# li-kunyi/CUT3R-SLAM

Measured on AMD Instinct MI355X. Metric: frames/sec (ViT pointmap + covisibility-graph tracking step) on 640x480, higher is better.
Workload: dtype f16

## Files before the change

### cut3r_slam_amd/_lib.py

```python
from __future__ import annotations

import ctypes as C
import os

_HERE = os.path.dirname(os.path.abspath(__file__))
LIB_PATH = os.path.join(_HERE, "libcut3r_hip.so")

c_void_p, c_int, c_float, c_ll = C.c_void_p, C.c_int, C.c_float, C.c_longlong


class GemmDesc(C.Structure):
    _fields_ = [
        ("A", c_void_p), ("B", c_void_p), ("C", c_void_p), ("bias", c_void_p), ("res1", c_void_p), ("res2", c_void_p),
        ("M", c_int), ("N", c_int), ("K", c_int), ("lda", c_int), ("ldb", c_int), ("ldc", c_int), ("ldr1", c_int),
        ("ldr2", c_int),
        ("act", c_int), ("out_f16", c_int), ("res1_f16", c_int), ("res2_f16", c_int),
        ("batch", c_int),
        ("strideA", c_ll), ("strideB", c_ll), ("strideC", c_ll), ("strideBias", c_ll), ("strideR1", c_ll),
        ("strideR2", c_ll),
        ("conv_k", c_int), ("H", c_int), ("W", c_int), ("Cin", c_int), ("conv_stride", c_int), ("Ho", c_int),
        ("Wo", c_int), ("relu_in", c_int),
        ("shuf", c_int), ("shuf_cout", c_int), ("shuf_Hin", c_int), ("shuf_Win", c_int),
        ("tile", c_int), ("stages", c_int),
        ("rope_pos", c_void_p), ("rope_table", c_void_p), ("rope_cols", c_int), ("rope_pmin", c_int), ("rope_npos", c_int),
# ... 3 lines not shown
    ]


class LcTerm(C.Structure):
    _fields_ = [("a", c_void_p), ("c", c_void_p), ("mask", c_void_p), ("ia", c_int), ("ic", c_int), ("w", c_float), ("pad", c_int)]


SIGNATURES = {
    "cut3r_abi_version": [],
    "cut3r_rope2d": [c_void_p, c_int, c_void_p, c_int, c_int, c_int, c_int, c_ll, c_ll, c_ll, c_float, c_float, c_void_p],
    "cut3r_rope2d_qk": [c_void_p, c_void_p, c_int, c_void_p, c_int, c_int, c_int, c_int, c_ll, c_ll, c_ll, c_ll, c_float, c_float,
                        c_void_p],
    "cut3r_rope2d_tab": [c_void_p, c_void_p, c_ll, c_ll, c_void_p, c_void_p, c_ll, c_ll, c_int, c_int, c_void_p, c_int, c_int, c_float,
                         c_float, c_void_p],
    "cut3r_layernorm": [c_void_p, c_int, c_void_p, c_void_p, c_float, c_int, c_int, c_void_p, c_int, c_void_p, c_int,
                        c_void_p, c_void_p, c_void_p],
    "cut3r_layernorm_dual": [c_void_p, c_int, c_void_p, c_void_p, c_void_p, c_int, c_void_p, c_void_p, c_void_p, c_int, c_float, c_int,
                             c_int, c_void_p],
    "cut3r_gemm_f16": [C.POINTER(GemmDesc), c_void_p],
    "cut3r_gemm_tile_for": [C.POINTER(GemmDesc)],
    "cut3r_gemm_f16_pair": [C.POINTER(GemmDesc), C.POINTER(GemmDesc), c_void_p],
    "cut3r_rope2d_table": [c_void_p, c_int, c_int, c_int, c_float, c_float, c_void_p],
    "cut3r_gemv_f16w": [c_void_p, c_int, c_void_p, c_int, c_void_p, c_void_p, c_int, c_int, c_int, c_int, c_int,
                        c_void_p, c_int, c_int, c_void_p],
    "cut3r_attention_variant": [c_int],
    "cut3r_attention_f16": [c_void_p, c_void_p, c_void_p, c_void_p, c_int, c_int, c_int, c_int, c_int,
                            c_ll, c_ll, c_ll, c_ll, c_ll, c_ll, c_ll, c_ll, c_float, c_void_p],
    "cut3r_im2col_patch": [c_void_p, c_int, c_int, c_int, c_int, c_int, c_int, c_void_p, c_void_p],
    "cut3r_cast_f32_f16": [c_void_p, c_int, c_void_p, c_int, c_int, c_int, c_void_p],
    "cut3r_colmean": [c_void_p, c_int, c_int, c_int, c_void_p, c_void_p],
    "cut3r_colmean_batched": [c_void_p, c_int, c_ll, c_int, c_int, c_int, c_void_p, c_ll, c_void_p],
    "cut3r_upsample2x_nhwc": [c_void_p, c_void_p, c_int, c_int, c_int, c_int, c_void_p],
    "cut3r_dpt_final": [c_void_p, c_int, c_int, c_void_p, c_void_p, c_int, c_void_p, c_void_p, c_void_p],
    "cut3r_postprocess_pts": [c_void_p, c_int, c_int, c_int, c_void_p, c_void_p, c_void_p],
    "cut3r_postprocess_pose": [c_void_p, c_int, c_void_p, c_void_p],
    "cut3r_patch_overlap": [c_void_p, c_void_p, c_int, c_int, c_float, c_void_p, c_void_p, c_void_p],
    "cut3r_patch_overlap_chain": [c_void_p, c_void_p, c_int, c_int, c_int, c_float, C.c_double, c_void_p, c_void_p, c_void_p, c_void_p,
                                  c_void_p, c_void_p],
    "cut3r_overlap_fwd": [c_void_p, c_int, C.POINTER(c_float), c_float, c_void_p, c_int, c_float, c_float, c_float, c_float,
                          c_int, c_int, c_int, c_void_p, c_void_p],
    "cut3r_overlap_bwd": [c_void_p, c_int, c_int, c_int, c_int, c_void_p, c_float, c_float, c_float, c_float, c_int, c_int,
                          c_void_p, c_void_p],
    "cut3r_window_update": [c_void_p, c_void_p, c_int, c_int, c_int, C.POINTER(c_float), c_float, c_int, c_void_p, c_void_p, c_void_p,
                            c_void_p, c_int, c_int, c_void_p, C.POINTER(c_float), c_int, c_int, c_float, c_float, c_float, c_float,
                            c_void_p, c_int, c_void_p, c_void_p],
    "cut3r_logdepth_accum": [c_void_p, c_void_p, c_int, c_void_p, c_void_p],
    "cut3r_resize_linear_u8": [c_void_p, c_int, c_int, c_int, c_void_p, c_int, c_int, c_int, c_void_p],
    "cut3r_mfma_probe": [c_void_p, c_int, c_int, c_int, c_void_p, c_void_p, c_void_p],
    "cut3r_remap_linear_u8": [c_void_p, c_int, c_int, c_int, c_void_p, c_void_p, c_void_p, c_int, c_int, c_void_p],
    "cut3r_align_view": [c_void_p, c_void_p, c_int, c_int, C.POINTER(c_float), c_float, c_int, c_void_p, c_void_p,
                         c_void_p, c_void_p],
    "cut3r_logdepth_sum": [c_void_p, c_void_p, c_int, c_void_p, c_void_p],
    "cut3r_lie_unary": [c_int, c_int, c_void_p, c_void_p, c_int, c_void_p],
    "cut3r_lie_unary_bwd": [c_int, c_int, c_void_p, c_void_p, c_void_p, c_int, c_void_p],
    "cut3r_lie_mul": [c_int, c_void_p, c_void_p, c_void_p, c_int, c_void_p],
    "cut3r_lie_mul_bwd": [c_int, c_void_p, c_void_p, c_void_p, c_void_p, c_void_p, c_int, c_void_p],
    "cut3r_lie_act": [c_int, c_void_p, c_void_p, c_void_p, c_int, c_int, c_int, c_void_p],
    "cut3r_lie_act_bwd": [c_int, c_void_p, c_void_p, c_void_p, c_void_p, c_void_p, c_int, c_int, c_int, c_void_p],
    "cut3r_lie_adj": [c_int, c_void_p, c_void_p, c_void_p, c_int, c_int, c_void_p],
    "cut3r_lc_workspace_floats": [c_int, c_int],
    "cut3r_lc_optimize": [c_void_p, c_void_p, c_ll, c_void_p, c_void_p, c_void_p, c_int, c_int, c_ll, c_int, c_float,
                          c_void_p, c_void_p, c_void_p, c_void_p, c_void_p, c_void_p, c_void_p],
    "cut3r_lc_optimize_terms": [c_void_p, c_int, c_int, c_int, c_int, c_float, c_void_p, c_void_p, c_void_p, c_void_p, c_void_p, c_void_p,
                                c_void_p],
    "cut3r_transform_submaps": [c_void_p, c_void_p, c_int, c_ll, c_void_p],
    "cut3r_corr_index_forward": [c_void_p, c_void_p, c_void_p, c_int, c_int, c_int, c_int, c_int, c_int, c_void_p],
# ... 85 lines not shown
```

### cut3r_slam_amd/csrc/elementwise.hip

```cpp
#include "common.h"
#include "../../include/cut3r_hip.h"

namespace {

template <typename T> struct alignas(4 * sizeof(T)) Vec4 { T v[4]; };

template <typename T>
__global__ __launch_bounds__(256) void rope2d_kernel(T* __restrict__ tok, T* __restrict__ tok2, const int64_t* __restrict__ pos,
                                                     int N, int H, int D, long long sB, long long sN, long long sH, long long sB2,
                                                     long long sN2, float base, float fwd) {
    __shared__ float cs[2][2][64];
    const int t = blockIdx.x;
    const int b = t / N, n = t - b * N;
    const int Q = D >> 2;
    if (threadIdx.x < 2 * Q) {
        const int X = threadIdx.x / Q, q = threadIdx.x - X * Q;
        const float inv = fwd / powf(base, (float)q / (float)Q);
        const float fr = (float)pos[(size_t)t * 2 + X] * inv;
        cs[X][0][q] = cosf(fr);
        cs[X][1][q] = sinf(fr);
    }
    __syncthreads();
    const int Q4 = Q >> 2;
    const int per_tensor = H * 2 * Q4;
    const int total = tok2 ? 2 * per_tensor : per_tensor;
    for (int w = threadIdx.x; w < total; w += blockDim.x) {
        const int which = w / per_tensor;
        int r = w - which * per_tensor;
        const int h = r / (2 * Q4);
        r -= h * 2 * Q4;
        const int X = r / Q4, c = r - X * Q4;
        T* base_p = which ? (tok2 + (size_t)b * sB2 + (size_t)n * sN2) : (tok + (size_t)b * sB + (size_t)n * sN);
        T* pu = base_p + (size_t)h * sH + X * 2 * Q + 4 * c;
// ... 360 lines not shown
        } else {
            const float eps = 1e-6f;
            float o[3] = {a0, a1, a2};
#pragma unroll
            for (int e = 0; e < 3; e++) {
                float sg = 1.0f / (1.0f + expf(-o[e]));
                pts[3 * p + e] = ((sg * (1 - 2 * eps) + eps) - 0.5f) * 2.0f;
            }
        }
    }
}

__global__ __launch_bounds__(256) void dpt_final_coalesced_kernel(const h16* __restrict__ in, int P, int Cin, const float* __restrict__ w,
                                                                  const float* __restrict__ bsv, int mode, float* __restrict__ pts,
                                                                  float* __restrict__ conf) {
    const int nout = mode == 0 ? 4 : 3;
    const int lane = threadIdx.x & 63;
    const int lpp = Cin >> 3;
    const int ppw = 64 / lpp;
    const int sub = lane / lpp, chunk = lane - sub * lpp;
    float wr[4][8];
#pragma unroll
    for (int o = 0; o < 4; o++)
#pragma unroll
        for (int e = 0; e < 8; e++) wr[o][e] = o < nout ? w[o * Cin + chunk * 8 + e] : 0.f;
    const float b0 = bsv[0], b1 = bsv[1], b2 = bsv[2], b3 = nout == 4 ? bsv[3] : 0.f;
    const size_t wave_global = (blockIdx.x * (size_t)blockDim.x + threadIdx.x) >> 6;
    const size_t nwaves = ((size_t)gridDim.x * blockDim.x) >> 6;
    for (size_t p0 = wave_global * ppw; p0 < (size_t)P; p0 += nwaves * ppw) {
        const size_t p = p0 + sub;
        float a0 = 0.f, a1 = 0.f, a2 = 0.f, a3 = 0.f;
        if (p < (size_t)P) {
            const half8_t v = *reinterpret_cast<const half8_t*>(in + p * Cin + chunk * 8);
#pragma unroll
            for (int e = 0; e < 8; e++) {
                const float xv = (float)v[e];
                a0 = fmaf(xv, wr[0][e], a0);
                a1 = fmaf(xv, wr[1][e], a1);
                a2 = fmaf(xv, wr[2][e], a2);
                a3 = fmaf(xv, wr[3][e], a3);
            }
        }
        for (int o = lpp >> 1; o > 0; o >>= 1) {
            a0 += __shfl_xor(a0, o, 64);
            a1 += __shfl_xor(a1, o, 64);
            a2 += __shfl_xor(a2, o, 64);
            a3 += __shfl_xor(a3, o, 64);
        }
        if (chunk == 0 && p < (size_t)P) {
            a0 += b0; a1 += b1; a2 += b2; a3 += b3;
            if (mode == 0) {
                act_pts_conf(a0, a1, a2, a3, true, false, pts, conf, p);
            } else {
                const float eps = 1e-6f;
                const float o3[3] = {a0, a1, a2};
#pragma unroll
                for (int e = 0; e < 3; e++) {
                    const float sg = 1.0f / (1.0f + expf(-o3[e]));
                    pts[3 * p + e] = ((sg * (1 - 2 * eps) + eps) - 0.5f) * 2.0f;
                }
            }
        }
    }
}

__global__ __launch_bounds__(256) void postprocess_pts_kernel(const float* __restrict__ raw, int P, int nch, int pos_z,
                                                              float* __restrict__ pts, float* __restrict__ conf) {
    for (size_t p = blockIdx.x * (size_t)blockDim.x + threadIdx.x; p < (size_t)P; p += (size_t)gridDim.x * blockDim.x) {
        const float* r = raw + p * nch;
        act_pts_conf(r[0], r[1], r[2], nch > 3 ? r[3] : 0.f, nch > 3, pos_z != 0, pts, conf, p);
    }
}

__global__ void postprocess_pose_kernel(const float* __restrict__ raw, int B, float* __restrict__ out) {
    const int b = blockIdx.x * blockDim.x + threadIdx.x;
    if (b >= B) return;
    const float* r = raw + b * 7;
    const float d = sqrtf(r[0] * r[0] + r[1] * r[1] + r[2] * r[2]);
    const float sc = expm1f(d) / fmaxf(d, 1e-8f);
    float qn = sqrtf(r[3] * r[3] + r[4] * r[4] + r[5] * r[5] + r[6] * r[6]);
    qn = fmaxf(qn, 1e-12f);
    float q[4] = {r[3] / qn, r[4] / qn, r[5] / qn, r[6] / qn};
    const float sg = q[0] < 0.f ? -1.f : 1.f;
    out[b * 7 + 0] = r[0] * sc; out[b * 7 + 1] = r[1] * sc; out[b * 7 + 2] = r[2] * sc;
    for (int e = 0; e < 4; e++) out[b * 7 + 3 + e] = sg * q[e];
// ... 241 lines not shown
```

### cut3r_slam_amd/csrc/gemm.hip

```cpp
#include <cstdlib>
#include "common.h"
#include "../../include/cut3r_hip.h"

namespace {

constexpr int BK = 64;
constexpr int KCH = BK / 8;

struct GemmArgs {
    const h16* A; const h16* B; void* C;
    const float* bias; const void* res1; const void* res2;
    int M, N, K, lda, ldb, ldc, ldr1, ldr2;
    int act, out_f16, res1_f16, res2_f16;
    long long sA, sB, sC, sBias, sR1, sR2;
    int conv_k, H, W, Cin, cstride, Ho, Wo, relu_in;
    int shuf, shuf_cout, shuf_Hin, shuf_Win;
    int swz;
    int prio;
    const long long* rope_pos; const float* rope_table; int rope_cols, rope_pmin, rope_npos, rope_d;
    const float* ln_stats; const float* ln_c; int ln_nslab; float ln_eps;
    float* stats_out; h16* out16; int ld16;
};

DEVINL half8_t relu8(half8_t v) {
#pragma unroll
    for (int i = 0; i < 8; i++) v[i] = v[i] > (h16)0 ? v[i] : (h16)0;
    return v;
}

__device__ __attribute__((aligned(16))) unsigned char g_zero16[16];

template <int N>
DEVINL void wait_vmcnt() { asm volatile("s_waitcnt vmcnt(%0)" ::"n"(N) : "memory"); }
template <int NL, int MAXF>
DEVINL void wait_tiles_in_flight(int fl) {
    static_assert(MAXF * NL <= 63, "vmcnt is a 6-bit counter");
    if constexpr (MAXF >= 6) { if (fl >= 6) { wait_vmcnt<6 * NL>(); return; } }
    if constexpr (MAXF >= 5) { if (fl == 5) { wait_vmcnt<5 * NL>(); return; } }
    if constexpr (MAXF >= 4) { if (fl == 4) { wait_vmcnt<4 * NL>(); return; } }
    if constexpr (MAXF >= 3) { if (fl == 3) { wait_vmcnt<3 * NL>(); return; } }
    if constexpr (MAXF >= 2) { if (fl == 2) { wait_vmcnt<2 * NL>(); return; } }
    if constexpr (MAXF >= 1) { if (fl == 1) { wait_vmcnt<NL>(); return; } }
    wait_vmcnt<0>();
}

DEVINL f32x4 load_res4(const void* res, int is_f16, size_t off) {
    if (is_f16) {
        const half4_t rv = *reinterpret_cast<const half4_t*>((const h16*)res + off);
        return f32x4{(float)rv[0], (float)rv[1], (float)rv[2], (float)rv[3]};
    }
    return *reinterpret_cast<const f32x4*>((const float*)res + off);
}
DEVINL f32x4 fused_finish4(const GemmArgs& g, f32x4 v, const f32x4& b4, bool has_bias, const f32x4& r1, const f32x4& r2) {
    if (has_bias) v += b4;
// ... 331 lines not shown
                fb[j] = *reinterpret_cast<const half8_t*>(sb + r * (BK * 2) + ((ch ^ (r & 7)) << 4));
            }
            if (g.prio) __builtin_amdgcn_s_setprio(1);
#pragma unroll
            for (int i = 0; i < MT; i++)
#pragma unroll
                for (int j = 0; j < NT; j++)
                    acc[i][j] = __builtin_amdgcn_mfma_f32_16x16x32_f16(fa[i], fb[j], acc[i][j], 0, 0, 0);
            if (g.prio) __builtin_amdgcn_s_setprio(0);
        }
        if (++stage == NSTAGE) stage = 0;
    }
    __syncthreads();

    float* cs = reinterpret_cast<float*>(smem);
    const float* lnp = reinterpret_cast<const float*>(smem + LNP_OFF);
    if (g.ln_stats && tid < BM) {
        float* w = reinterpret_cast<float*>(smem + LNP_OFF) + 2 * tid;
        w[0] = ln_rs; w[1] = ln_rm;
    }
    const float* bias = g.bias ? g.bias + (size_t)z * g.sBias : nullptr;
    constexpr int TPR = BN / 4;
    constexpr int RPP = NTHR / TPR;
    constexpr int ITER = (EPI_ROWS + RPP - 1) / RPP;
    constexpr int PF = (MT * NT >= 12) ? 2 : (ITER < 4 ? ITER : 4);
    const int c4 = (tid % TPR) * 4;
    const int gn = n0 + c4;
    const int r0 = tid / TPR;
    const bool col_ok = gn < N && tid < RPP * TPR;
    const bool plain = !g.shuf && g.rope_cols == 0;
    const f32x4 zero4 = {0.f, 0.f, 0.f, 0.f};
    f32x4 b4 = zero4;
    if (bias && col_ok && plain) b4 = *reinterpret_cast<const f32x4*>(bias + gn);
    if constexpr (EPI != 0) {
        constexpr bool F16OUT = EPI != 3, RES = (EPI == 3 || EPI == 5);
        const int gnc = col_ok ? gn : 0;
        const f32x4 bb = *reinterpret_cast<const f32x4*>(bias + gnc);
#pragma unroll
        for (int p = 0; p < EPI_PASSES; p++) {
            f32x4 rv[ITER], sv[ITER];
            if (RES) {
#pragma unroll
                for (int i = 0; i < ITER; i++) {
                    const size_t gm = (size_t)min(m0 + p * EPI_ROWS + r0 + i * RPP, M - 1);
                    if (EPI == 3) {
                        rv[i] = *reinterpret_cast<const f32x4*>((const float*)g.res1 + (size_t)z * g.sR1 + gm * g.ldr1 + gnc);
                    } else {
                        const half4_t h1 = *reinterpret_cast<const half4_t*>((const h16*)g.res1 + (size_t)z * g.sR1 + gm * g.ldr1 + gnc);
                        rv[i] = f32x4{(float)h1[0], (float)h1[1], (float)h1[2], (float)h1[3]};
                        if (g.res2) {
                            const half4_t h2 = *reinterpret_cast<const half4_t*>((const h16*)g.res2 + (size_t)z * g.sR2 + gm * g.ldr2 + gnc);
                            sv[i] = f32x4{(float)h2[0], (float)h2[1], (float)h2[2], (float)h2[3]};
                        }
                    }
                }
            }
            if (p > 0) __syncthreads();
#pragma unroll
            for (int i = 0; i < MT; i++)
#pragma unroll
                for (int j = 0; j < NT; j++)
#pragma unroll
                    for (int e = 0; e < 4; e++) {
                        const int r = wm * WM + i * 16 + fq * 4 + e - p * EPI_ROWS;
                        const int c = wn * WN + j * 16 + fr;
                        if (EPI_PASSES == 1 || (r >= 0 && r < EPI_ROWS)) cs[r * CPAD + c] = acc[i][j][e];
// ... 1013 lines not shown
            if (ep == 3 && ns8 == 6) hipLaunchKernelGGL((gemm_kernel<64, 64, 6, 2, 4, 1, 3>), grid, dim3(512), 0, s, g);
            else if (ep == 3 && ns8 == 4) hipLaunchKernelGGL((gemm_kernel<64, 64, 4, 2, 4, 1, 3>), grid, dim3(512), 0, s, g);
            else if (ep == 3) hipLaunchKernelGGL((gemm_kernel<64, 64, 3, 2, 4, 1, 3>), grid, dim3(512), 0, s, g);
            else if (am == 1) hipLaunchKernelGGL((gemm_kernel<64, 64, 3, 2, 4, 1>), grid, dim3(512), 0, s, g);
            else if (am == 2) hipLaunchKernelGGL((gemm_kernel<64, 64, 3, 2, 4, 2>), grid, dim3(512), 0, s, g);
            else hipLaunchKernelGGL((gemm_kernel<64, 64, 3, 2, 4>), grid, dim3(512), 0, s, g);
        }
        else if (d->stages == 4) hipLaunchKernelGGL((gemm_kernel<64, 64, 4>), grid, dim3(256), 0, s, g);
        else {
            const int am = d->stages == 0 ? tile_addr_mode(g) : 0;
            const int ep = am == 1 ? gemm256_epi_mode(g) : 0;
            if (g.stats_out && ep != 3) return CUT3R_ERR_ARG;
            static const int ns4 = [] { const char* e = getenv("CUT3R_GEMM64_STAGES"); return e ? atoi(e) : 3; }();
#define CUT3R_T64(NS)                                                                                                   \
    do {                                                                                                                 \
        if (ep == 1) hipLaunchKernelGGL((gemm_kernel<64, 64, NS, 2, 2, 1, 1>), grid, dim3(256), 0, s, g);                \
        else if (ep == 2) hipLaunchKernelGGL((gemm_kernel<64, 64, NS, 2, 2, 1, 2>), grid, dim3(256), 0, s, g);           \
        else if (ep == 3) hipLaunchKernelGGL((gemm_kernel<64, 64, NS, 2, 2, 1, 3>), grid, dim3(256), 0, s, g);           \
        else hipLaunchKernelGGL((gemm_kernel<64, 64, NS, 2, 2, 1>), grid, dim3(256), 0, s, g);                           \
    } while (0)
            if (am == 1 && ns4 == 6) CUT3R_T64(6);
            else if (am == 1 && ns4 == 4) CUT3R_T64(4);
            else if (am == 1) CUT3R_T64(3);
#undef CUT3R_T64
            else if (am == 2) hipLaunchKernelGGL((gemm_kernel<64, 64, 3, 2, 2, 2>), grid, dim3(256), 0, s, g);
            else hipLaunchKernelGGL((gemm_kernel<64, 64, 3>), grid, dim3(256), 0, s, g);
        }
    } else {
        return CUT3R_ERR_ARG;
    }
    return cut3r_check_launch();
}

extern "C" int cut3r_gemm_f16_pair(const cut3r_gemm_desc* d0, const cut3r_gemm_desc* d1, void* stream) {
    if (!d0 || !d1) return CUT3R_ERR_ARG;
    GemmPairArgs a;
    int rc = fill_args(d0, a.p[0]);
    if (rc != CUT3R_OK) return rc;
    rc = fill_args(d1, a.p[1]);
    if (rc != CUT3R_OK) return rc;
    for (const cut3r_gemm_desc* d : {d0, d1})
        if (d->conv_k == 3 || d->shuf || d->relu_in || (d->batch > 1)) return CUT3R_ERR_ARG;
    if (d0->N != d1->N || d0->K != d1->K) return CUT3R_ERR_ARG;
    hipStream_t s = (hipStream_t)stream;
    const bool special = d0->ln_stats || d1->ln_stats || d0->stats_out || d1->stats_out || a.p[0].rope_cols || a.p[1].rope_cols;
    int tile = d0->tile;
    if (tile == 0) {
        const long long t256 = (long long)((d0->M + 255) / 256 + (d1->M + 255) / 256) * ((d0->N + 255) / 256);
        const long long rounds = (t256 + 255) / 256;
        const bool fills = rounds == 1 || t256 * 100 >= rounds * 256 * 85;
        const long long t128 = (long long)((d0->M + 127) / 128 + (d1->M + 127) / 128) * ((d0->N + 127) / 128);
        tile = ((d0->N & 255) == 0 && t256 >= 128 && fills && !special) ? 256 : ((t128 >= 128 && !special) ? 128 : 64);
    }
    if (special && tile != 64) return CUT3R_ERR_ARG;
    if (tile == 64) {
        const int n0 = ((d0->N + 63) / 64) * ((d0->M + 63) / 64), n1 = ((d1->N + 63) / 64) * ((d1->M + 63) / 64);
        a.nblk0 = n0;
        a.p[0].swz = a.p[1].swz = 1;
        const bool am = tile_addr_mode(a.p[0]) == 1 && tile_addr_mode(a.p[1]) == 1;
        const int e0 = gemm256_epi_mode(a.p[0]), e1 = gemm256_epi_mode(a.p[1]);
        const int ep = (am && e0 == e1 && (e0 == 1 || e0 == 2 || e0 == 3)) ? e0 : 0;
        if ((d0->stats_out || d1->stats_out) && ep != 3) return CUT3R_ERR_ARG;
        const dim3 grid(n0 + n1);
        if (d0->K >= 2048) {
            if (ep == 3) hipLaunchKernelGGL((gemm_pair_kernel<64, 64, 3, 2, 4, 1, 3>), grid, dim3(512), 0, s, a);
            else if (am) hipLaunchKernelGGL((gemm_pair_kernel<64, 64, 3, 2, 4, 1, 0>), grid, dim3(512), 0, s, a);
// ... 36 lines not shown
```

### cut3r_slam_amd/model.py

```python
from __future__ import annotations

import gc

import math
import re
from dataclasses import dataclass
from typing import Dict, List, Optional

import torch

from . import ops
from .config import Cut3rConfig, production_config, state_dict_schema

F16, F32 = torch.float16, torch.float32


@dataclass
class ARCroco3DStereoOutput:
    ress: Optional[List[dict]] = None
    views: Optional[List[dict]] = None


class _Lin:

# ... 6 lines not shown
            w2 = torch.cat([w2, torch.zeros(pad, w2.shape[1])], 0)
            if b is not None:
                b = torch.cat([b.to(F32), torch.zeros(pad)], 0)
        self.w = w2.to(device=dev, dtype=F16).contiguous()
        self.b = b.to(device=dev, dtype=F32).contiguous() if b is not None else None
        self.npad = n + pad
        self.k = self.w.shape[1]


class Cut3rModel:
    def __init__(self, cfg: Cut3rConfig, state_dict: Dict[str, torch.Tensor], device="cuda:0", minimal: bool = False):
        self.cfg = cfg
        self.device = torch.device(device)
        self.minimal = minimal
        schema = state_dict_schema(cfg)
        missing = [k for k in schema if k not in state_dict]
        if missing:
            raise KeyError(f"state_dict is missing {len(missing)} tensors, e.g. {missing[:4]}")
        for k, shp in schema.items():
            if tuple(state_dict[k].shape) != tuple(shp):
                raise ValueError(f"{k}: shape {tuple(state_dict[k].shape)} != schema {tuple(shp)}")
        self._buf: Dict[tuple, torch.Tensor] = {}
        self._graphs: Dict[tuple, tuple] = {}
        import os as _os
        self.use_graphs = _os.environ.get("CUT3R_GRAPHS", "1") != "0"
        self.dual_stream = _os.environ.get("CUT3R_DUAL_STREAM", "1") != "0"
        self.dual_ln = _os.environ.get("CUT3R_DUAL_LN", "1") != "0"
        self.pair_gemm = _os.environ.get("CUT3R_PAIR_GEMM", "0") != "0"
        self.pair_rows = int(_os.environ.get("CUT3R_PAIR_ROWS", "0"))
        self.fused_rope = int(_os.environ.get("CUT3R_FUSED_ROPE", "1"))
        self.rope48_rows = int(_os.environ.get("CUT3R_ROPE48_ROWS", "0"))
        self.head_overlap = _os.environ.get("CUT3R_HEAD_OVERLAP", "1") != "0"
        self.head_chunk = max(1, int(_os.environ.get("CUT3R_HEAD_CHUNK", "28")))
        self.ln_fold = int(_os.environ.get("CUT3R_LN_FOLD", "1"))
        self._head_stream = None
        self._side = None
        self._head_side = None
        self.kv_fork = _os.environ.get("CUT3R_KV_FORK", "0") != "0"
        self.kv_fork_rows = int(_os.environ.get("CUT3R_KV_FORK_ROWS", "2048"))
        self._kv_streams = None
        self._prep(state_dict)

    @classmethod
    def from_state_dict(cls, cfg, sd, device="cuda:0", **kw):
        return cls(cfg, sd, device, **kw)

    @classmethod
    def from_pretrained(cls, path: str, config: Optional[Cut3rConfig] = None, device="cuda:0", **kw):
        import argparse
        import os
        if not os.path.isfile(path):
            raise FileNotFoundError(f"{path}: no checkpoint (this runtime never fetches from a hub)")
        with torch.serialization.safe_globals([argparse.Namespace]):
            ckpt = torch.load(path, map_location="cpu", weights_only=True)
        sd = ckpt["model"] if "model" in ckpt else ckpt
        sd = {(k[7:] if k.startswith("module.") else k): v for k, v in sd.items()}
        if not any(k.startswith("dec_blocks_state") for k in sd):
            for k in list(sd):
                if k.startswith("dec_blocks"):
                    sd[k.replace("dec_blocks", "dec_blocks_state")] = sd[k]
        if config is None:
            config = production_config()
            args = getattr(ckpt.get("args", None), "model", "") if isinstance(ckpt, dict) else ""
            config = _config_from_ctor_string(args, config)
        return cls(config, sd, device, **kw)

# ... 459 lines not shown
        B, H, W, _ = x.shape
        Ho, Wo = (H - 1) // stride + 1, (W - 1) // stride + 1
        out = self.buf(tag or name, (B, Ho, Wo, L.npad), F16)
        return ops.conv3x3_nhwc(x, L.w, out, L.b, stride, relu_in, act, res1, res2)

    def _conv1(self, x, name, tag=None):
        L = self.w[name]
        B, H, W, Cc = x.shape
        out = self.buf(tag or name, (B, H, W, L.npad), F16)
        ops.linear(x.view(-1, Cc), L.w, out.view(-1, L.npad), L.b)
        return out

    def _convT(self, x, name):
        L = self.w[name]
        B, H, W, Cc = x.shape
        cout = L.npad // (L.s * L.s)
        out = self.buf(name, (B, H * L.s, W * L.s, cout), F16)
        return ops.conv_transpose_nhwc(x, L.w, out, L.b, L.s)

    def _up2(self, x, tag):
        B, H, W, Cc = x.shape
        return ops.upsample2x(x, self.buf(tag, (B, 2 * H, 2 * W, Cc), F16))

    def _rcu(self, x, p, res2=None):
        t = self._conv3(x, p + ".conv1", relu_in=True, act=2)
        return self._conv3(t, p + ".conv2", res1=x, res2=res2)

    def _fusion(self, p, x0, x1=None):
        out = x0 if x1 is None else self._rcu(x1, p + ".resConfUnit1", res2=x0)
        out = self._rcu(out, p + ".resConfUnit2")
        out = self._up2(out, p + ".up")
        return self._conv1(out, p + ".out_conv")

    def _dpt(self, p, toks16: List[torch.Tensor], B, nh, nw):
        a = p + ".act_postprocess"
        t = [x.view(B, nh, nw, -1) for x in toks16]
        l0 = self._convT(self._conv1(t[0], a + ".0.0"), a + ".0.1")
        l1 = self._convT(self._conv1(t[1], a + ".1.0"), a + ".1.1")
        l2 = self._conv1(t[2], a + ".2.0")
        l3 = self._conv3(self._conv1(t[3], a + ".3.0"), a + ".3.1", stride=2)
        L = [self._conv3(l, f"{p}.scratch.layer_rn.{i}") for i, l in enumerate((l0, l1, l2, l3))]
        p4 = self._fusion(p + ".scratch.refinenet4", L[3])
        if p4.shape[1] != L[2].shape[1] or p4.shape[2] != L[2].shape[2]:
            p4 = p4[:, : L[2].shape[1], : L[2].shape[2]].contiguous()
        p3 = self._fusion(p + ".scratch.refinenet3", p4, L[2])
        p2 = self._fusion(p + ".scratch.refinenet2", p3, L[1])
        p1 = self._fusion(p + ".scratch.refinenet1", p2, L[0])
        o = self._conv3(p1, p + ".head.0")
        o = self._up2(o, p + ".head.up")
        o = self._conv3(o, p + ".head.2", act=2)
        return o

    def _dpt_pts(self, p, toks16, B, nh, nw, H, W, key_pts, key_conf, res, out=None):
        o = self._dpt(p, toks16, B, nh, nw)
        if out is None:
            pts = torch.empty((B, H, W, 3), dtype=F32, device=self.device)
            conf = torch.empty((B, H, W), dtype=F32, device=self.device)
        else:
            pts, conf = out
        ops.dpt_final(o.view(B * H * W, -1), self.w[p + ".head.4.w"], self.w[p + ".head.4.b"], 0, pts, conf)
        if res is not None:
            res[key_pts], res[key_conf] = pts, conf

    @torch.no_grad()
    def forward_window(self, imgs: torch.Tensor, return_taps: bool = False):
        if self.use_graphs and not return_taps:
            return self._graphed("win", lambda x: self._forward_window(x, False), imgs.contiguous())
        return self._forward_window(imgs, return_taps)

    @torch.no_grad()
    def encode_batch(self, imgs: torch.Tensor) -> torch.Tensor:
        if self.use_graphs:
            feat, _, _ = self._graphed("enc", self._encode, imgs.contiguous())
            return feat.clone()
        return self._encode(imgs)[0]

    @torch.no_grad()
    def decode_window(self, feats: torch.Tensor, H: int, W: int):
        if self.use_graphs:
            return self._graphed(("dec", H, W), lambda f: self._forward_window(None, False, feats=f, hw=(H, W)), feats.contiguous())
        return self._forward_window(None, False, feats=feats, hw=(H, W))

    def _forward_window(self, imgs, return_taps: bool = False, feats=None, hw=None):
        P = self.cfg.patch_size
        if feats is None:
            V, _, H, W = imgs.shape
            feat, feat16, _ = self._encode(imgs)
            res, taps = self._decode(feat[None], feat16[None], H, W, return_taps)
        else:
            H, W = hw
            res, taps = self._decode(feats[None], None, H, W, return_taps)
            V = feats.shape[0]
        preds = [{k: v[i:i + 1] for k, v in res.items()} for i in range(V)]
# ... 117 lines not shown
                        self._dec_block("decs", f"dec_blocks_state.{l}", s_a, a, pos_state, pos_img, cfg.state_dec_num_heads, s_b, Wn, pre_ln=pre,
                                        xs=xsa, ys=xa, os_=xsb)
                        self._dec_block("deci", f"dec_blocks.{l}", a, s_a, pos_img, pos_state, cfg.dec_num_heads, b, Wn, pre_ln=pre, xs=xa, ys=xsa, os_=xb)
                s_a, s_b = s_b, s_a
                a, b = b, a
                if l + 1 == h1 or l + 1 == h2:
                    tk = tok1 if l + 1 == h1 else tok2
                    tk[:, i].copy_(a.view(Wn, N + 1, D)[:, 1:])
            if not dead_tail:
                self._ln(s_a, "dec_norm_state", out32=s_b)
            new_state = s_b
            self._ln(a, "dec_norm", out16=dn16, out32=dn32)
            dn16v, dn32v = dn16.view(Wn, N + 1, D), dn32.view(Wn, N + 1, D)
            tok3[:, i].copy_(dn16v[:, 1:])
            if tok3_32 is not None:
                tok3_32[:, i].copy_(dn32v[:, 1:])
            pose_tok[:, i].copy_(dn32v[:, 0])
            pose_tok16[:, i].copy_(dn16v[:, 0])
            if not dead_tail:
                self._mem_update(mem[cm], g16, dn32v[:, 0], mem[cm ^ 1], Wn)
                cm ^= 1
            if head_fork:
                cur = torch.cuda.current_stream()
                self._head_stream.wait_stream(cur)
                with torch.cuda.stream(self._head_stream):
                    for c0 in range(0, Wn, self.head_chunk):
                        c1 = min(Wn, c0 + self.head_chunk)
                        nb = c1 - c0
                        tk = []
                        for name, src, dim in (("f", feat16, E), ("t1", tok1, D), ("t2", tok2, D), ("t3", tok3, D)):
                            t = self.buf("head.view." + name, (nb, N, dim), F16)
                            t.copy_(src[c0:c1, i])
                            tk.append(t.view(nb * N, dim))
                        pv = self.buf("head.view.pts", (nb, H, W, 3), F32)
                        cv = self.buf("head.view.conf", (nb, H, W), F32)
                        self._dpt_pts("downstream_head.dpt_self", tk, nb, nh, nw, H, W, None, None, None, out=(pv, cv))
                        head_pts.view(Wn, V, H, W, 3)[c0:c1, i].copy_(pv)
                        head_conf.view(Wn, V, H, W)[c0:c1, i].copy_(cv)
            cs = 0 if new_state is st[0] else 1
            if return_taps:
                states.append((new_state.view(Wn, S, D)[0].clone(), mem[cm].view(Wn, msz, 2 * D)[0].clone()))
        if return_taps:
            taps["states"] = states

        BV = Wn * V
        h = "downstream_head"
        ph = self.buf("head.pose_h", (BV, self.w[h + ".pose_head.mlp.fc1"].npad), F16)
        self._linear(pose_tok16.view(BV, D), h + ".pose_head.mlp.fc1", ph, act=1)
        praw = self.buf("head.pose_raw", (BV, 8), F32)
        self._linear(ph, h + ".pose_head.mlp.fc2", praw)
        pose = torch.empty((BV, 7), dtype=F32, device=dev)
        ops.postprocess_pose(praw[:, :7].contiguous(), pose)
        res: Dict[str, torch.Tensor] = {"camera_pose": pose}
        toks = [feat16.reshape(BV * N, E), tok1.view(BV * N, D), tok2.view(BV * N, D), tok3.view(BV * N, D)]
        if head_fork:
            torch.cuda.current_stream().wait_stream(self._head_stream)
            res["pts3d_in_self_view"], res["conf_self"] = head_pts, head_conf
        elif cfg.head_type == "dpt":
            pts = torch.empty((BV, H, W, 3), dtype=F32, device=dev)
            conf = torch.empty((BV, H, W), dtype=F32, device=dev)
            for c0 in range(0, BV, 8):
                c1 = min(BV, c0 + 8)
                tk = [t.view(BV, N, -1)[c0:c1].reshape((c1 - c0) * N, -1) for t in toks]
                self._dpt_pts(h + ".dpt_self", tk, c1 - c0, nh, nw, H, W, None, None, None, out=(pts[c0:c1], conf[c0:c1]))
            res["pts3d_in_self_view"], res["conf_self"] = pts, conf
        else:
            self._linear_head(h + ".proj", tok3.view(BV * N, D), BV, nh, nw, True, "pts3d_in_self_view", "conf_self", res)
        if not self.minimal:
            posBV = pos1.expand(BV, -1, -1).contiguous()
            self._cross_heads(toks, tok3_32.view(BV, N, D), pose_tok.view(BV, D), posBV, BV, nh, nw, H, W, res)
        return res, taps
# ... 112 lines not shown
```

### cut3r_slam_amd/ops.py

```python
from __future__ import annotations

import ctypes as C
import os
from typing import Optional

import torch

from . import _lib
from ._lib import GemmDesc, check

F16, F32 = torch.float16, torch.float32


def _stream():
    return C.c_void_p(torch.cuda.current_stream().cuda_stream)


def _p(t: Optional[torch.Tensor]):
    return C.c_void_p(t.data_ptr()) if t is not None else C.c_void_p(0)


def _req(cond, msg):
    if not cond:
        raise ValueError(msg)
# ... 262 lines not shown
    if bias is not None:
        _req(bias.dtype == F32 and bias.shape == (Z, N) and bias.stride(1) == 1, "bias [Z,N]")
        d.strideBias = bias.stride(0)
    if res1 is not None:
        _req(res1.shape == (Z, M, N) and res1.stride(2) == 1 and res1.dtype in (F16, F32), "res1 [Z,M,N]")
        d.res1, d.ldr1, d.res1_f16, d.strideR1 = res1.data_ptr(), res1.stride(1), int(res1.dtype == F16), res1.stride(0)
    d.M, d.N, d.K, d.lda, d.ldb, d.ldc = M, N, K, A.stride(1), W.stride(1), out.stride(1)
    d.batch, d.strideA, d.strideB, d.strideC = Z, A.stride(0), W.stride(0), out.stride(0)
    lib = _lib.load()
    check(lib.cut3r_gemm_f16(C.byref(d), _stream()), f"cut3r_gemm_f16 batched Z={Z} M={M} N={N} K={K}")
    return out


def conv3x3_nhwc(x, Wk, out, bias=None, stride=1, relu_in=False, act=0, res1=None, res2=None, tile=0):
    _cuda(x, Wk, out, bias, res1, res2)
    _req(x.dtype == F16 and x.dim() == 4 and x.is_contiguous(), "x must be contiguous NHWC fp16")
    Bn, H, Wd, Cin = x.shape
    Cout = Wk.shape[0]
    Ho, Wo = (H + 2 - 3) // stride + 1, (Wd + 2 - 3) // stride + 1
    _req(Wk.dtype == F16 and Wk.shape == (Cout, 9 * Cin) and Wk.is_contiguous(), "Wk must be fp16 [Cout, 9*Cin]")
    _req(out.shape == (Bn, Ho, Wo, Cout) and out.is_contiguous() and out.dtype in (F16, F32), "bad conv output")
    M = Bn * Ho * Wo
    r1 = res1.reshape(M, Cout) if res1 is not None else None
    r2 = res2.reshape(M, Cout) if res2 is not None else None
    d = GemmDesc()
    _fill_common(d, x, Wk, out, bias, r1, r2, act, tile)
    d.M, d.N, d.K, d.lda, d.ldb, d.ldc = M, Cout, 9 * Cin, Cin, 9 * Cin, Cout
    d.conv_k, d.H, d.W, d.Cin, d.conv_stride, d.Ho, d.Wo, d.relu_in = 3, H, Wd, Cin, stride, Ho, Wo, int(relu_in)
    lib = _lib.load()
    check(lib.cut3r_gemm_f16(C.byref(d), _stream()), f"cut3r_gemm_f16(conv3x3) M={M} N={Cout} K={9*Cin}")
    return out


def conv_transpose_nhwc(x, Wt, out, bias, s):
    _cuda(x, Wt, out, bias)
    Bn, H, Wd, Cin = x.shape
    Cout = Wt.shape[0] // (s * s)
    _req(x.dtype == F16 and x.is_contiguous() and Wt.dtype == F16 and Wt.is_contiguous(), "fp16 contiguous inputs")
    _req(Wt.shape == (s * s * Cout, Cin) and out.shape == (Bn, H * s, Wd * s, Cout) and out.is_contiguous(), "bad shapes")
    _req(bias is not None and bias.numel() == Cout, "bias [Cout]")
    d = GemmDesc()
    _fill_common(d, x, Wt, out, bias, None, None, 0, 0)
    d.M, d.N, d.K, d.lda, d.ldb, d.ldc = Bn * H * Wd, s * s * Cout, Cin, Cin, Cin, Cout
    d.shuf, d.shuf_cout, d.shuf_Hin, d.shuf_Win = s, Cout, H, Wd
    lib = _lib.load()
    check(lib.cut3r_gemm_f16(C.byref(d), _stream()), "cut3r_gemm_f16(convT)")
    return out


def gemv(X, W, out, bias=None, act=0, res=None, silu_in=False):
    _cuda(X, W, out, bias, res)
    _req(X.dtype == F32 and W.dtype == F16 and out.dtype == F32, "dtypes: X fp32, W fp16, out fp32")
    M, K = X.shape
    N = W.shape[0]
    _req(W.shape[1] == K and out.shape == (M, N) and X.stride(1) == 1 and W.stride(1) == 1 and out.stride(1) == 1, "shapes")
    if bias is not None:
        _req(bias.dtype == F32 and bias.numel() == N, "bias")
    if res is not None:
        _req(res.dtype == F32 and res.shape == (M, N) and res.stride(1) == 1, "res")
    lib = _lib.load()
    check(lib.cut3r_gemv_f16w(_p(X), X.stride(0), _p(W), W.stride(0), _p(bias), _p(out), out.stride(0), M, N, K, act,
                              _p(res), res.stride(0) if res is not None else 0, int(silu_in), _stream()), "cut3r_gemv_f16w")
    return out


def attention(q, k, v, out, scale):
# ... 444 lines not shown
```

### include/cut3r_hip.h

```cpp
#ifndef CUT3R_HIP_H
#define CUT3R_HIP_H
#include <stdint.h>
#ifdef __cplusplus
extern "C" {
#endif

int cut3r_abi_version(void);

int cut3r_rope2d(void* tokens, int dtype, const int64_t* positions, int B, int N, int H, int D,
                 long long sB, long long sN, long long sH, float base, float fwd, void* stream);
int cut3r_rope2d_qk(void* q, void* k, int dtype, const int64_t* positions, int B, int N, int H, int D, long long q_sB,
                    long long q_sN, long long k_sB, long long k_sN, float base, float fwd, void* stream);

int cut3r_rope2d_tab(void* t0, const int64_t* pos0, long long ntok0, long long stride0, void* t1, const int64_t* pos1, long long ntok1,
                     long long stride1, int H, int D, const float* table, int pmin, int npos, float base, float fwd, void* stream);

int cut3r_layernorm(const float* x, int ldx, const float* gamma, const float* beta, float eps, int M, int C,
                    void* y16, int ld16, float* y32, int ld32, const float* mod_scale, const float* mod_shift,
                    void* stream);
int cut3r_layernorm_dual(const float* x, int ldx, const float* g1, const float* b1, void* y1, int ld1, const float* g2,
                         const float* b2, void* y2, int ld2, float eps, int M, int C, void* stream);

typedef struct cut3r_gemm_desc {
    const void* A;
// ... 18 lines not shown
    const float* rope_table;
    int rope_cols, rope_pmin, rope_npos;
    int rope_d;
    const float* ln_stats;
    const float* ln_colsum;
    int ln_nslab;
    float ln_eps;
    float* stats_out;
    void* out16;
    int ld16;
} cut3r_gemm_desc;
int cut3r_gemm_f16(const cut3r_gemm_desc* d, void* stream);
int cut3r_rope2d_table(float* table, int pmin, int npos, int Q, float base, float fwd, void* stream);
int cut3r_gemm_tile_for(const cut3r_gemm_desc* d);
int cut3r_gemm_f16_pair(const cut3r_gemm_desc* d0, const cut3r_gemm_desc* d1, void* stream);

int cut3r_gemv_f16w(const float* X, int ldx, const void* W, int ldw, const float* bias, float* Y, int ldy,
                    int M, int N, int K, int act, const float* res, int ldr, int silu_in, void* stream);

int cut3r_attention_f16(const void* q, const void* k, const void* v, void* out, int B, int H, int Nq, int Nk, int D,
                        long long q_sb, long long q_sn, long long k_sb, long long k_sn, long long v_sb, long long v_sn,
                        long long o_sb, long long o_sn, float scale, void* stream);

int cut3r_attention_variant(int v);

int cut3r_im2col_patch(const void* img, int u8, int B, int C, int H, int W, int P, void* out, void* stream);
int cut3r_cast_f32_f16(const float* x, int ldx, void* y, int ldy, int M, int C, void* stream);
int cut3r_colmean(const float* x, int ldx, int M, int C, float* y, void* stream);
int cut3r_colmean_batched(const float* x, int B, long long stride_x, int ldx, int M, int C, float* y, long long stride_y, void* stream);

int cut3r_upsample2x_nhwc(const void* in, void* out, int B, int H, int W, int C, void* stream);
int cut3r_dpt_final(const void* in, int P, int Cin, const float* w, const float* b, int mode, float* pts, float* conf,
                    void* stream);
int cut3r_postprocess_pts(const float* raw, int P, int nch, int pos_z, float* pts, float* conf, void* stream);
int cut3r_postprocess_pose(const float* raw, int B, float* out, void* stream);

int cut3r_patch_overlap(const float* feat0, const float* feat1, int N, int C, float thr, void* ws, int32_t* count,
                        void* stream);
int cut3r_patch_overlap_chain(const float* feat_last, const float* feats, int B, int N, int C, float thr_sim, double thr_ratio,
                              const int32_t* forced_host, void* ws, int32_t* state, int32_t* counts, int32_t* decisions,
                              void* stream);

int cut3r_overlap_fwd(const float* pm, int N, const float* P_host, float s_align, const float* w2c, int B, float fx, float fy,
                      float cx, float cy, int W, int H, int clamp_z ,
                      int32_t* counts, void* stream);
int cut3r_overlap_bwd(const float* pms, int B, int N, int grp, int grp_stride, const float* w2c, float fx, float fy, float cx,
                      float cy, int W, int H, int32_t* counts, void* stream);

int cut3r_window_update(const float* pts, const float* conf, int V, int H, int W, const float* P_host, float s, int ds,
                        float* pm_ds, float* conf_ds, float* depth, const float* store, int grp, int grp_stride,
                        float* w2c, const float* w2c_new_host, int t0, int first, float fx, float fy, float cx, float cy,
                        int32_t* counts, int ldc, double* lsum_reset, void* stream);

int cut3r_logdepth_accum(const float* prev_depth, const float* pts, int n, double* out, void* stream);

int cut3r_align_view(const float* pts, const float* conf, int H, int W, const float* P_host, float s, int ds,
                     float* pm_ds, float* conf_ds, float* depth, void* stream);
int cut3r_logdepth_sum(const float* prev_depth, const float* pts, int n, double* out, void* stream);

int cut3r_lie_unary(int group, int op, const float* in, float* out, int n, void* stream);
int cut3r_lie_unary_bwd(int group, int op, const float* in, const float* grad_out, float* grad_in, int n, void* stream);
int cut3r_lie_mul(int group, const float* x, const float* y, float* out, int n, void* stream);
int cut3r_lie_mul_bwd(int group, const float* x, const float* y, const float* grad_out, float* grad_x, float* grad_y, int n,
                      void* stream);
int cut3r_lie_act(int group, const float* x, const float* p, float* out, int n, int P, int pd, void* stream);
int cut3r_lie_act_bwd(int group, const float* x, const float* p, const float* grad_out, float* grad_x, float* grad_p, int n, int P,
// ... 144 lines not shown
```

Baseline: 5812.

## Fuse DPT head 3x3 conv with final 1x1 projection and pts/conf activation

Adds a GEMM epilogue variant that applies bias+ReLU to the 128-channel 3x3 conv output tile in shared memory, then does the 4-output 1x1 projection and the pts/conf activation directly. The fp16 full-resolution intermediate is no longer written to and read back from global memory. The head path now writes straight into strided per-view output slices, which drops the staging buffers and copies. In exchange the kernel is pinned to a 192x128 tile and pays extra shared-memory passes and shuffle reductions in the epilogue.

```diff
diff --git a/cut3r_slam_amd/_lib.py b/cut3r_slam_amd/_lib.py
--- a/cut3r_slam_amd/_lib.py
+++ b/cut3r_slam_amd/_lib.py
@@ -59,6 +59,7 @@
     "cut3r_colmean_batched": [c_void_p, c_int, c_ll, c_int, c_int, c_int, c_void_p, c_ll, c_void_p],
     "cut3r_upsample2x_nhwc": [c_void_p, c_void_p, c_int, c_int, c_int, c_int, c_void_p],
     "cut3r_dpt_final": [c_void_p, c_int, c_int, c_void_p, c_void_p, c_int, c_void_p, c_void_p, c_void_p],
+    "cut3r_conv3x3_dpt_final": [C.POINTER(GemmDesc), c_void_p, c_void_p, c_void_p, c_void_p, c_ll, c_ll, c_void_p],
     "cut3r_postprocess_pts": [c_void_p, c_int, c_int, c_int, c_void_p, c_void_p, c_void_p],
     "cut3r_postprocess_pose": [c_void_p, c_int, c_void_p, c_void_p],
     "cut3r_patch_overlap": [c_void_p, c_void_p, c_int, c_int, c_float, c_void_p, c_void_p, c_void_p],
diff --git a/cut3r_slam_amd/csrc/dpt_math.h b/cut3r_slam_amd/csrc/dpt_math.h
--- /dev/null
+++ b/cut3r_slam_amd/csrc/dpt_math.h
@@ -0,0 +1,33 @@
+#pragma once
+#include "common.h"
+
+DEVINL void dpt_dot8(const float (&x)[8], const float (&w)[4][8], float& a0, float& a1, float& a2, float& a3) {
+#pragma clang fp contract(off)
+#pragma unroll
+    for (int e = 0; e < 8; e++) {
+        a0 = fmaf(x[e], w[0][e], a0);
+        a1 = fmaf(x[e], w[1][e], a1);
+        a2 = fmaf(x[e], w[2][e], a2);
+        a3 = fmaf(x[e], w[3][e], a3);
+    }
+}
+
+DEVINL void dpt_pixel_sum(int lpp, float& a0, float& a1, float& a2, float& a3) {
+    for (int o = lpp >> 1; o > 0; o >>= 1) {
+        a0 += __shfl_xor(a0, o, 64);
+        a1 += __shfl_xor(a1, o, 64);
+        a2 += __shfl_xor(a2, o, 64);
+        a3 += __shfl_xor(a3, o, 64);
+    }
+}
+
+DEVINL void dpt_pts_conf(float x, float y, float z, float c, float* __restrict__ pts3, float* __restrict__ conf1) {
+#pragma clang fp contract(off)
+    const float d = sqrtf(fmaf(y, y, x * x) + z * z);
+    const float dc = fmaxf(d, 1e-8f);
+    const float e = expm1f(d);
+    pts3[0] = x / dc * e;
+    pts3[1] = y / dc * e;
+    pts3[2] = z / dc * e;
+    *conf1 = 1.0f + expf(c);
+}
diff --git a/cut3r_slam_amd/csrc/elementwise.hip b/cut3r_slam_amd/csrc/elementwise.hip
--- a/cut3r_slam_amd/csrc/elementwise.hip
+++ b/cut3r_slam_amd/csrc/elementwise.hip
@@ -1,4 +1,5 @@
 #include "common.h"
+#include "dpt_math.h"
 #include "../../include/cut3r_hip.h"
 
 namespace {
@@ -425,25 +426,16 @@
         float a0 = 0.f, a1 = 0.f, a2 = 0.f, a3 = 0.f;
         if (p < (size_t)P) {
             const half8_t v = *reinterpret_cast<const half8_t*>(in + p * Cin + chunk * 8);
-#pragma unroll
-            for (int e = 0; e < 8; e++) {
-                const float xv = (float)v[e];
-                a0 = fmaf(xv, wr[0][e], a0);
-                a1 = fmaf(xv, wr[1][e], a1);
-                a2 = fmaf(xv, wr[2][e], a2);
-                a3 = fmaf(xv, wr[3][e], a3);
-            }
-        }
-        for (int o = lpp >> 1; o > 0; o >>= 1) {
-            a0 += __shfl_xor(a0, o, 64);
-            a1 += __shfl_xor(a1, o, 64);
-            a2 += __shfl_xor(a2, o, 64);
-            a3 += __shfl_xor(a3, o, 64);
-        }
+            float xv[8];
+#pragma unroll
+            for (int e = 0; e < 8; e++) xv[e] = (float)v[e];
+            dpt_dot8(xv, wr, a0, a1, a2, a3);
+        }
+        dpt_pixel_sum(lpp, a0, a1, a2, a3);
         if (chunk == 0 && p < (size_t)P) {
             a0 += b0; a1 += b1; a2 += b2; a3 += b3;
             if (mode == 0) {
-                act_pts_conf(a0, a1, a2, a3, true, false, pts, conf, p);
+                dpt_pts_conf(a0, a1, a2, a3, pts + 3 * p, conf + p);
             } else {
                 const float eps = 1e-6f;
                 const float o3[3] = {a0, a1, a2};
diff --git a/cut3r_slam_amd/csrc/gemm.hip b/cut3r_slam_amd/csrc/gemm.hip
--- a/cut3r_slam_amd/csrc/gemm.hip
+++ b/cut3r_slam_amd/csrc/gemm.hip
@@ -1,5 +1,6 @@
 #include <cstdlib>
 #include "common.h"
+#include "dpt_math.h"
 #include "../../include/cut3r_hip.h"
 
 namespace {
@@ -20,6 +21,7 @@
     const long long* rope_pos; const float* rope_table; int rope_cols, rope_pmin, rope_npos, rope_d;
     const float* ln_stats; const float* ln_c; int ln_nslab; float ln_eps;
     float* stats_out; h16* out16; int ld16;
+    const float* dpt_w; const float* dpt_b; float* dpt_pts; float* dpt_conf; long long dpt_sp, dpt_sc; int dpt_hw;
 };
 
 DEVINL half8_t relu8(half8_t v) {
@@ -417,6 +419,55 @@
     const f32x4 zero4 = {0.f, 0.f, 0.f, 0.f};
     f32x4 b4 = zero4;
     if (bias && col_ok && plain) b4 = *reinterpret_cast<const f32x4*>(bias + gn);
+    if constexpr (EPI == 7) {
+        static_assert(BN == 128, "a tile row must hold all 128 channels of a pixel");
+        constexpr int PPI = NTHR / 16;
+        static_assert(EPI_ROWS % PPI == 0, "uniform trip count (the butterfly needs every lane)");
+        const int chunk = tid & 15, sub = tid >> 4;
+        float wr[4][8], bb8[8];
+#pragma unroll
+        for (int o = 0; o < 4; o++)
+#pragma unroll
+            for (int e = 0; e < 8; e++) wr[o][e] = g.dpt_w[o * 128 + chunk * 8 + e];
+#pragma unroll
+        for (int e = 0; e < 8; e++) bb8[e] = bias[chunk * 8 + e];
+        const float d0 = g.dpt_b[0], d1 = g.dpt_b[1], d2 = g.dpt_b[2], d3 = g.dpt_b[3];
+#pragma unroll
+        for (int p = 0; p < EPI_PASSES; p++) {
+            if (p > 0) __syncthreads();
+#pragma unroll
+            for (int i = 0; i < MT; i++)
+#pragma unroll
+                for (int j = 0; j < NT; j++)
+#pragma unroll
+                    for (int e = 0; e < 4; e++) {
+                        const int r = wm * WM + i * 16 + fq * 4 + e - p * EPI_ROWS;
+                        const int c = wn * WN + j * 16 + fr;
+                        if (EPI_PASSES == 1 || (r >= 0 && r < EPI_ROWS)) cs[r * CPAD + c] = acc[i][j][e];
+                    }
+            __syncthreads();
+            for (int r = sub; r < EPI_ROWS; r += PPI) {
+                const int gm = m0 + p * EPI_ROWS + r;
+                const f32x4 lo = *reinterpret_cast<const f32x4*>(cs + r * CPAD + chunk * 8);
+                const f32x4 hi = *reinterpret_cast<const f32x4*>(cs + r * CPAD + chunk * 8 + 4);
+                float xv[8];
+#pragma unroll
+                for (int e = 0; e < 8; e++) {
+                    const float v = fmaxf((e < 4 ? lo[e] : hi[e - 4]) + bb8[e], 0.f);
+                    xv[e] = (float)(h16)v;
+                }
+                float a0 = 0.f, a1 = 0.f, a2 = 0.f, a3 = 0.f;
+                dpt_dot8(xv, wr, a0, a1, a2, a3);
+                dpt_pixel_sum(16, a0, a1, a2, a3);
+                if (chunk == 0 && gm < M) {
+                    a0 += d0; a1 += d1; a2 += d2; a3 += d3;
+                    const int b = gm / g.dpt_hw, px = gm - b * g.dpt_hw;
+                    dpt_pts_conf(a0, a1, a2, a3, g.dpt_pts + (size_t)b * g.dpt_sp + 3 * (size_t)px, g.dpt_conf + (size_t)b * g.dpt_sc + px);
+                }
+            }
+        }
+        return;
+    }
     if constexpr (EPI != 0) {
         constexpr bool F16OUT = EPI != 3, RES = (EPI == 3 || EPI == 5);
         const int gnc = col_ok ? gn : 0;
@@ -1496,6 +1547,28 @@
     return cut3r_check_launch();
 }
 
+extern "C" int cut3r_conv3x3_dpt_final(const cut3r_gemm_desc* d, const float* w4, const float* b4, float* pts, float* conf,
+                                       long long pts_stride, long long conf_stride, void* stream) {
+    if (!d) return CUT3R_ERR_ARG;
+    cut3r_gemm_desc dd = *d;
+    dd.C = const_cast<void*>(dd.A);
+    GemmArgs g;
+    const int rc = fill_args(&dd, g);
+    if (rc != CUT3R_OK) return rc;
+    if (d->conv_k != 3 || d->conv_stride != 1 || d->N != 128 || d->act != 2 || !d->out_f16 || !d->bias || ((uintptr_t)d->bias & 15) || d->relu_in ||
+        d->res1 || d->res2 || d->shuf || d->rope_pos || d->ln_stats || d->stats_out || batch_of(d) != 1 || !w4 || !b4 || !pts || !conf ||
+        pts_stride < 0 || conf_stride < 0)
+        return CUT3R_ERR_ARG;
+    g.dpt_w = w4; g.dpt_b = b4; g.dpt_pts = pts; g.dpt_conf = conf;
+    g.dpt_sp = pts_stride; g.dpt_sc = conf_stride; g.dpt_hw = d->Ho * d->Wo;
+    g.swz = 1;
+    const dim3 grid((unsigned)((d->M + 191) / 192));
+    hipStream_t s = (hipStream_t)stream;
+    if (tile_addr_mode(g) == 2) hipLaunchKernelGGL((gemm_kernel<192, 128, 2, 4, 2, 2, 7>), grid, dim3(512), 0, s, g);
+    else hipLaunchKernelGGL((gemm_kernel<192, 128, 2, 4, 2, 0, 7>), grid, dim3(512), 0, s, g);
+    return cut3r_check_launch();
+}
+
 extern "C" int cut3r_gemm_f16_pair(const cut3r_gemm_desc* d0, const cut3r_gemm_desc* d1, void* stream) {
     if (!d0 || !d1) return CUT3R_ERR_ARG;
     GemmPairArgs a;
diff --git a/cut3r_slam_amd/model.py b/cut3r_slam_amd/model.py
--- a/cut3r_slam_amd/model.py
+++ b/cut3r_slam_amd/model.py
@@ -62,6 +62,7 @@
         self.rope48_rows = int(_os.environ.get("CUT3R_ROPE48_ROWS", "0"))
         self.head_overlap = _os.environ.get("CUT3R_HEAD_OVERLAP", "1") != "0"
         self.head_chunk = max(1, int(_os.environ.get("CUT3R_HEAD_CHUNK", "28")))
+        self.dpt_fused = _os.environ.get("CUT3R_DPT_FUSED", "1") != "0"
         self.ln_fold = int(_os.environ.get("CUT3R_LN_FOLD", "1"))
         self._head_stream = None
         self._side = None
@@ -587,7 +588,7 @@
         out = self._up2(out, p + ".up")
         return self._conv1(out, p + ".out_conv")
 
-    def _dpt(self, p, toks16: List[torch.Tensor], B, nh, nw):
+    def _dpt(self, p, toks16: List[torch.Tensor], B, nh, nw, head2=True):
         a = p + ".act_postprocess"
         t = [x.view(B, nh, nw, -1) for x in toks16]
         l0 = self._convT(self._conv1(t[0], a + ".0.0"), a + ".0.1")
@@ -603,17 +604,24 @@
         p1 = self._fusion(p + ".scratch.refinenet1", p2, L[0])
         o = self._conv3(p1, p + ".head.0")
         o = self._up2(o, p + ".head.up")
+        if not head2:
+            return o
         o = self._conv3(o, p + ".head.2", act=2)
         return o
 
     def _dpt_pts(self, p, toks16, B, nh, nw, H, W, key_pts, key_conf, res, out=None):
-        o = self._dpt(p, toks16, B, nh, nw)
         if out is None:
             pts = torch.empty((B, H, W, 3), dtype=F32, device=self.device)
             conf = torch.empty((B, H, W), dtype=F32, device=self.device)
         else:
             pts, conf = out
-        ops.dpt_final(o.view(B * H * W, -1), self.w[p + ".head.4.w"], self.w[p + ".head.4.b"], 0, pts, conf)
+        if self.dpt_fused:
+            o = self._dpt(p, toks16, B, nh, nw, head2=False)
+            L = self.w[p + ".head.2"]
+            ops.conv3x3_dpt_final(o, L.w, L.b, self.w[p + ".head.4.w"], self.w[p + ".head.4.b"], pts, conf)
+        else:
+            o = self._dpt(p, toks16, B, nh, nw)
+            ops.dpt_final(o.view(B * H * W, -1), self.w[p + ".head.4.w"], self.w[p + ".head.4.b"], 0, pts, conf)
         if res is not None:
             res[key_pts], res[key_conf] = pts, conf
 
@@ -797,11 +805,15 @@
                             t = self.buf("head.view." + name, (nb, N, dim), F16)
                             t.copy_(src[c0:c1, i])
                             tk.append(t.view(nb * N, dim))
-                        pv = self.buf("head.view.pts", (nb, H, W, 3), F32)
-                        cv = self.buf("head.view.conf", (nb, H, W), F32)
-                        self._dpt_pts("downstream_head.dpt_self", tk, nb, nh, nw, H, W, None, None, None, out=(pv, cv))
-                        head_pts.view(Wn, V, H, W, 3)[c0:c1, i].copy_(pv)
-                        head_conf.view(Wn, V, H, W)[c0:c1, i].copy_(cv)
+                        hp, hc = head_pts.view(Wn, V, H, W, 3)[c0:c1, i], head_conf.view(Wn, V, H, W)[c0:c1, i]
+                        if self.dpt_fused:
+                            self._dpt_pts("downstream_head.dpt_self", tk, nb, nh, nw, H, W, None, None, None, out=(hp, hc))
+                        else:
+                            pv = self.buf("head.view.pts", (nb, H, W, 3), F32)
+                            cv = self.buf("head.view.conf", (nb, H, W), F32)
+                            self._dpt_pts("downstream_head.dpt_self", tk, nb, nh, nw, H, W, None, None, None, out=(pv, cv))
+                            hp.copy_(pv)
+                            hc.copy_(cv)
             cs = 0 if new_state is st[0] else 1
             if return_taps:
                 states.append((new_state.view(Wn, S, D)[0].clone(), mem[cm].view(Wn, msz, 2 * D)[0].clone()))
diff --git a/cut3r_slam_amd/ops.py b/cut3r_slam_amd/ops.py
--- a/cut3r_slam_amd/ops.py
+++ b/cut3r_slam_amd/ops.py
@@ -318,6 +318,24 @@
     return out
 
 
+def conv3x3_dpt_final(x, Wk, bias, w4, b4, pts, conf):
+    _cuda(x, Wk, bias, w4, b4, pts, conf)
+    _req(x.dtype == F16 and x.dim() == 4 and x.is_contiguous(), "x must be contiguous NHWC fp16")
+    Bn, H, Wd, Cin = x.shape
+    _req(Wk.dtype == F16 and Wk.shape == (128, 9 * Cin) and Wk.is_contiguous(), "Wk must be fp16 [128, 9*Cin]")
+    _req(bias is not None and bias.dtype == F32 and bias.numel() == 128 and bias.is_contiguous(), "bias fp32 [128]")
+    _req(w4.dtype == F32 and w4.shape == (4, 128) and w4.is_contiguous() and b4.dtype == F32 and b4.numel() == 4, "head.4 w [4,128] / b [4]")
+    _req(pts.dtype == F32 and pts.shape == (Bn, H, Wd, 3) and pts[0].is_contiguous(), "pts fp32 [B,H,W,3], contiguous per image")
+    _req(conf.dtype == F32 and conf.shape == (Bn, H, Wd) and conf[0].is_contiguous(), "conf fp32 [B,H,W], contiguous per image")
+    d = GemmDesc()
+    _fill_common(d, x, Wk, x, bias, None, None, 2, 0)
+    d.M, d.N, d.K, d.lda, d.ldb, d.ldc = Bn * H * Wd, 128, 9 * Cin, Cin, 9 * Cin, 128
+    d.conv_k, d.H, d.W, d.Cin, d.conv_stride, d.Ho, d.Wo, d.relu_in = 3, H, Wd, Cin, 1, H, Wd, 0
+    lib = _lib.load()
+    check(lib.cut3r_conv3x3_dpt_final(C.byref(d), _p(w4), _p(b4), _p(pts), _p(conf), pts.stride(0), conf.stride(0), _stream()),
+          f"cut3r_conv3x3_dpt_final M={d.M} K={9*Cin}")
+
+
 def conv_transpose_nhwc(x, Wt, out, bias, s):
     _cuda(x, Wt, out, bias)
     Bn, H, Wd, Cin = x.shape
diff --git a/include/cut3r_hip.h b/include/cut3r_hip.h
--- a/include/cut3r_hip.h
+++ b/include/cut3r_hip.h
@@ -74,6 +74,8 @@
 int cut3r_upsample2x_nhwc(const void* in, void* out, int B, int H, int W, int C, void* stream);
 int cut3r_dpt_final(const void* in, int P, int Cin, const float* w, const float* b, int mode, float* pts, float* conf,
                     void* stream);
+int cut3r_conv3x3_dpt_final(const cut3r_gemm_desc* d, const float* w4, const float* b4, float* pts, float* conf,
+                            long long pts_stride, long long conf_stride, void* stream);
 int cut3r_postprocess_pts(const float* raw, int P, int nch, int pos_z, float* pts, float* conf, void* stream);
 int cut3r_postprocess_pose(const float* raw, int B, float* out, void* stream);
 
```

Result: no change. 5816 (median of 4 runs) (+0.1%).
